# genome/ibwa

Hardware: AMD Instinct MI355X
Metric: reads/s `ibwa aln` GRCh37-sized 100bp, achieved HBM GB/s vs peak (higher is better)
Workload: dtype u32

## Files before the change

ibwa_amd/csrc/aln.hip:

```cpp
#include <hip/hip_runtime.h>
#include <stdint.h>
#include "engine.h"
#include "occ.h"

namespace ibwa {

namespace {


struct Fetch {
  uint4 ck, bk, sk, cl, bl, sl;
  uint32_t offk, offl;
  bool kneg;
};

__device__ __forceinline__ void fetch_pair(const IndexView &ix, uint32_t k, uint32_t l, Fetch &f) {
  f.kneg = (k == 0xFFFFFFFFu);
  uint32_t kk = f.kneg ? 0u : bwt_kk(ix, k);
  uint32_t ll = bwt_kk(ix, l);
  const uint4 *pk = ix.blk + (size_t)(kk >> 7) * 4;
  const uint4 *pl = ix.blk + (size_t)(ll >> 7) * 4;
  f.offk = kk & 127;
  f.offl = ll & 127;
  f.ck = pk[0];
// ... 84 lines not shown
}

__device__ __forceinline__ void occ4x2_from(const Fetch &f, uint32_t ck[4], uint32_t cl[4]) {
  if (f.kneg) {
    ck[0] = ck[1] = ck[2] = ck[3] = 0;
  } else {
    occ4_from(f.ck, f.bk, f.sk, f.offk, ck);
  }
  occ4_from(f.cl, f.bl, f.sl, f.offl, cl);
}

__device__ __forceinline__ uint32_t strand_base(uint32_t c, int a, bool comp) {
  return (a == 1 && comp && c < 4) ? 3u - c : c;
}

struct RecOut {
  uint32_t *words;
  uint32_t off, acc;
  __device__ __forceinline__ void put(uint32_t byte) {
    acc |= byte << (8 * (off & 3));
    if ((off & 3) == 3) {
      words[off >> 2] = acc;
      acc = 0;
    }
    ++off;
  }
  __device__ __forceinline__ void flush() {
    if (off & 3) words[off >> 2] = acc;
    acc = 0;
  }
};

__device__ __forceinline__ uint32_t rec_byte(uint2 a, uint2 b, uint32_t pa, uint32_t pb, bool first, uint32_t clamp,
                                             int nb) {
  const uint32_t ea = !first && a.x == pa, eb = !first && b.x == pb;
  return (a.y < clamp ? a.y : clamp) | ea << (nb - 1) | ((b.y < clamp ? b.y : clamp) | eb << (nb - 1)) << nb;
}

struct WChain {
  uint32_t k, l, bid;
  uint32_t mode, t, wi, w, w2;
};

struct WLoad {
  Fetch1 f;
  uint32_t q, w, w2, wi;
  bool tl;
};

__device__ __forceinline__ bool win_has(const WChain &h, uint32_t p) {
  return h.wi != 0xFFFFFFFFu && p >= 16u * h.wi && p - 16u * h.wi < 32u;
}

__device__ __forceinline__ void wchain_load(const IndexView &ix, const uint32_t *sa, const uint32_t *tx,
                                            const WChain &h, uint32_t c, WLoad &x, bool refresh) {
  fetch1(ix, h.k - 1, h.l, c & 3, c < 4 && h.mode != 2, x.f);
  x.q = 0;
  if (h.mode == 1) x.q = sa[h.k];
  const uint32_t p = h.t - 1u;
  x.tl = h.mode == 2 && h.t > 0 && (!win_has(h, p) || (refresh && !win_has(h, p >= 15u ? p - 15u : 0u)));
  x.wi = (p >= 15u ? p - 15u : 0u) >> 4;
  x.w = h.w;
  x.w2 = h.w2;
  if (x.tl) {
    x.w = tx[x.wi];
    x.w2 = tx[x.wi + 1];
  }
}

__device__ __forceinline__ void wchain_step(const IndexView &ix, bool jump, WChain &h, uint32_t c, const WLoad &x) {
  if (h.mode == 2) {
    if (x.tl) { h.w = x.w; h.w2 = x.w2; h.wi = x.wi; }
    const uint32_t p = h.t - 1u;
    const uint32_t tw = p - 16u * h.wi < 16u ? h.w : h.w2;
    if (h.t > 0 && c < 4 && ((tw >> (2 * (p & 15))) & 3u) == c) {
      --h.t;
    } else {
      h.k = 0; h.l = ix.seq_len; ++h.bid; h.mode = 0;
    }
    return;
  }
  bool reset = c > 3;
  if (c < 4) {
    uint32_t ok, ol;
    occ2_from1(x.f, c, ok, ol);
    h.k = l2of(ix, c) + ok + 1;
    h.l = l2of(ix, c) + ol;
    reset = h.k > h.l;
  }
  if (reset) { h.k = 0; h.l = ix.seq_len; ++h.bid; }
  if (h.mode == 1) {
    h.mode = reset ? 0u : 2u;
    h.t = x.q - 1u;
    h.wi = 0xFFFFFFFFu;
  } else if (jump && !reset && h.k == h.l) {
    h.mode = 1;
  }
}

__device__ __forceinline__ void width_pair(const IndexView ixa, const IndexView ixb, int L, const uint8_t *s, bool comp,
                                           uint2 *wa, uint2 *wb, uint32_t *lw = nullptr, RecOut *rec = nullptr,
                                           uint32_t clamp = 0, int nb = 4, uint32_t *rd = nullptr,
                                           const uint32_t *sa0 = nullptr, const uint32_t *sa1 = nullptr,
                                           const uint32_t *tx0 = nullptr, const uint32_t *tx1 = nullptr,
                                           const uint2 *lta = nullptr, const uint2 *ltb = nullptr, int tdep = 0) {
  WChain A{0u, ixa.seq_len, 0u, 0u, 0u, 0xFFFFFFFFu, 0u, 0u};
  WChain B{0u, ixb.seq_len, 0u, 0u, 0u, 0xFFFFFFFFu, 0u, 0u};
  uint32_t lwa = 0, lwb = 0;
  uint32_t pa = 0, pb = 0;
  constexpr int TMAX = 15;
  uint2 ta[TMAX], tb[TMAX];
  int da = 0, db = 0;
  if (tdep > 0) {
    const int D = L < tdep ? L : tdep;
    uint32_t xa = 0, xb = 0;
    int dn = D;
#pragma unroll
    for (int d = 0; d < TMAX; ++d) {
      ta[d] = tb[d] = make_uint2(1u, 0u);
      if (d < dn) {
// ... 14 lines not shown
      da += (d < dn && ta[d].x <= ta[d].y) ? 1 : 0;
      db += (d < dn && tb[d].x <= tb[d].y) ? 1 : 0;
    }
  }
  auto block = [&](int base, auto first) __attribute__((always_inline)) {
    constexpr bool FIRST = decltype(first)::value;
    uint2 ba[16], bb[16];
#pragma unroll
    for (int t = 0; t < 16; ++t) {
      const int i = base + t;
      if (i < L) {
        uint32_t ca = s[i];
        uint32_t cb = strand_base(ca, 1, comp);
        const bool tA = FIRST && t < TMAX && t < da, tB = FIRST && t < TMAX && t < db;
        WLoad xa, xb;
        if (!tA) wchain_load(ixa, sa0, tx0, A, ca, xa, t == 0);
        if (!tB) wchain_load(ixb, sa1, tx1, B, cb, xb, t == 0);
        if (FIRST && t < TMAX && tA) {
          A.k = ta[t < TMAX ? t : 0].x;
          A.l = ta[t < TMAX ? t : 0].y;
          if (t == da - 1 && sa0 != nullptr && A.k == A.l) A.mode = 1;
        } else {
          wchain_step(ixa, sa0 != nullptr, A, ca, xa);
        }
        if (FIRST && t < TMAX && tB) {
          B.k = tb[t < TMAX ? t : 0].x;
          B.l = tb[t < TMAX ? t : 0].y;
          if (t == db - 1 && sa1 != nullptr && B.k == B.l) B.mode = 1;
        } else {
          wchain_step(ixb, sa1 != nullptr, B, cb, xb);
        }
        ba[t] = make_uint2(A.l - A.k + 1, A.bid);
        lwa += 31 - __builtin_clz(A.l - A.k + 1);
        bb[t] = make_uint2(B.l - B.k + 1, B.bid);
        lwb += 31 - __builtin_clz(B.l - B.k + 1);
      }
    }
#pragma unroll
    for (int t = 0; t < 16; ++t)
      if (base + t < L) wa[base + t] = ba[t];
#pragma unroll
    for (int t = 0; t < 16; ++t)
      if (base + t < L) wb[base + t] = bb[t];
    if (rec) {
      uint32_t x = 0;
#pragma unroll
      for (int t = 0; t < 16; ++t)
        if (base + t < L) {
          rec->put(rec_byte(ba[t], bb[t], pa, pb, base + t == 0, clamp, nb));
          pa = ba[t].x;
          pb = bb[t].x;
          x |= ((uint32_t)s[base + t] & 3u) << (2 * t);
        }
      if (rd) rd[base >> 4] = x;
    }
  };
  if (L > 0) block(0, std::true_type{});
  for (int base = 16; base < L; base += 16) block(base, std::false_type{});
  wa[L] = make_uint2(0u, A.bid + 1);
  wb[L] = make_uint2(0u, B.bid + 1);
  if (rec) rec->put(rec_byte(wa[L], wb[L], pa, pb, L == 0, clamp, nb));
  if (lw) {
    lw[0] = lwa;
    lw[1] = lwb;
    lw[2] = A.bid;
    lw[3] = B.bid;
  }
}

__global__ void __launch_bounds__(256) k_width(AlnArgs A) {
  const int64_t lane = (int64_t)blockIdx.x * blockDim.x + threadIdx.x;
  if (lane >= A.n) return;
  const int64_t r = A.ids ? A.ids[lane] : lane;
  const int L = (int)A.len[r];
  const uint8_t *s = A.seq + A.off[r];
  const bool comp = A.o.mode & MODE_COMPREAD;
  const uint32_t *sa0 = A.jsa[0], *sa1 = A.jsa[1], *tx0 = A.jtxt[0], *tx1 = A.jtxt[1];
  const int tdep = A.ltab[0] ? (int)min(A.tab_k + 1u, 15u) : 0;
  uint2 *w0 = A.wbuf + (uint64_t)lane * A.wstride;
  uint2 *w1 = w0 + A.wlen1;
  uint2 *sw0 = w1 + A.wlen1;
  uint2 *sw1 = sw0 + (A.o.seed_len + 1);
  if (A.nN) {
    uint32_t nN = 0;
    for (int j = 0; j < L; ++j) nN += s[j] > 3;
    A.nN[lane] = (uint16_t)(nN > 0xFFFFu ? 0xFFFFu : nN);
  }
  if (A.feat) {
    uint32_t f[4] = {0, 0, 0, 0}, g[4] = {0, 0, 0, 0};
    width_pair(A.ix[0], A.ix[1], L, s, comp, w0, w1, f);
    if (L > A.o.seed_len) width_pair(A.ix[0], A.ix[1], A.o.seed_len, s + (L - A.o.seed_len), comp, sw0, sw1, g);
    A.feat[lane * 4 + 0] = (uint16_t)(f[0] + f[1]);
    A.feat[lane * 4 + 1] = (uint16_t)(g[0] + g[1]);
    A.feat[lane * 4 + 2] = (uint16_t)(f[2] < f[3] ? f[2] : f[3]);
    A.feat[lane * 4 + 3] = (uint16_t)(g[2] < g[3] ? g[2] : g[3]);
    return;
  }
  if (A.cw) {
    uint32_t *rec = A.cw + (uint64_t)lane * A.cw_words;
    uint32_t nN = 0;
    for (int j = 0; j < L; ++j) nN += s[j] > 3;
    const int md = A.o.fnr_pos ? (int)A.maxdiff_tab[L] : A.o.max_diff;
    rec[0] = (uint32_t)L | (nN < 255u ? nN : 255u) << 16 | (uint32_t)md << 24;
    RecOut ro{rec + 1 + A.cw_rw, 0u, 0u};
    width_pair(A.ix[0], A.ix[1], L, s, comp, w0, w1, nullptr, &ro, (uint32_t)md + 1u, 4, rec + 1, sa0, sa1, tx0, tx1,
               A.ltab[0], A.ltab[1], tdep);
    while (ro.off < A.wlen1) ro.put(0u);
    if (L > A.o.seed_len)
      width_pair(A.ix[0], A.ix[1], A.o.seed_len, s + (L - A.o.seed_len), comp, sw0, sw1, nullptr, &ro,
                 (uint32_t)A.o.max_seed_diff + 1u, 3, nullptr, sa0, sa1, tx0, tx1, A.ltab[0], A.ltab[1], tdep);
    ro.flush();
    return;
  }
  width_pair(A.ix[0], A.ix[1], L, s, comp, w0, w1, nullptr, nullptr, 0, 4, nullptr, sa0, sa1, tx0, tx1, A.ltab[0],
             A.ltab[1], tdep);
  if (L > A.o.seed_len)
    width_pair(A.ix[0], A.ix[1], A.o.seed_len, s + (L - A.o.seed_len), comp, sw0, sw1, nullptr, nullptr, 0, 4,
               nullptr, sa0, sa1, tx0, tx1, A.ltab[0], A.ltab[1], tdep);
}

__device__ __forceinline__ bool match_exact_alt(const IndexView &ix, int i, const uint8_t *s, int a, bool comp,
                                                uint32_t &k0, uint32_t &l0) {
  uint32_t k = k0, l = l0;
  for (int j = i - 1; j >= 0; --j) {
    uint32_t c = strand_base(s[j], a, comp);
    if (c > 3) return false;
    Fetch1 f;
    fetch1(ix, k - 1, l, c, true, f);
    uint32_t ok, ol;
    occ2_from1(f, c, ok, ol);
    k = l2of(ix, c) + ok + 1;
    l = l2of(ix, c) + ol;
    if (k > l) return false;
// ... 213 lines not shown
  int64_t t = (int64_t)blockIdx.x * blockDim.x + threadIdx.x;
  if (t >= n) return;
  uint32_t o[4];
  occ4(ix, k[t], o);
  cnt[4 * t + 0] = o[0];
  cnt[4 * t + 1] = o[1];
  cnt[4 * t + 2] = o[2];
  cnt[4 * t + 3] = o[3];
}

}

hipError_t launch_width(const AlnArgs &a, int block, hipStream_t st) {
  if (a.n <= 0) return hipSuccess;
  uint64_t grid = (a.n + block - 1) / block;
  hipLaunchKernelGGL(k_width, dim3((unsigned)grid), dim3(block), 0, st, a);
  return hipGetLastError();
}

hipError_t launch_search(const AlnArgs &a, int block, hipStream_t st) {
  if (a.n <= 0) return hipSuccess;
  uint64_t grid = (a.n + block - 1) / block;
  hipLaunchKernelGGL(k_search, dim3((unsigned)grid), dim3(block), 0, st, a);
  return hipGetLastError();
}

hipError_t launch_occ4(const IndexView &ix, int64_t n, const uint32_t *k, uint32_t *cnt, hipStream_t st) {
  if (n <= 0) return hipSuccess;
  hipLaunchKernelGGL(k_occ4, dim3((unsigned)((n + 255) / 256)), dim3(256), 0, st, ix, n, k, cnt);
  return hipGetLastError();
}
// ... 3 lines not shown
```

ibwa_amd/csrc/engine.h:

```cpp
#pragma once
#include <hip/hip_runtime.h>
#include <stdint.h>
#include "occ.h"

namespace ibwa {

constexpr uint32_t NIL = 0xFFFFFFFFu;
constexpr uint32_t ST_STACK_OVERFLOW = 1u;
constexpr uint32_t ST_ALN_OVERFLOW = 2u;
constexpr uint32_t ST_BAD_SCORE = 4u;
constexpr uint32_t ST_HEAVY = 8u;

enum CounterSlot {
  CTR_CLAIM = 0,
  CTR_STREAM = 1,
  CTR_WIDE_STREAM = 2,
  CTR_HANDED_ON = 3,
  CTR_RESUMED = 5,
  CTR_TAIL_JUMPS = 7,
};
enum CoopNextSlot {
  CNEXT_POOL = 0,
  CNEXT_PSTORE = 1,
};

struct AlnOpt {
  int s_mm, s_gapo, s_gape, mode;
  int indel_end_skip, max_del_occ, max_entries;
  int fnr_pos;
  int max_diff;
  int max_gapo;
  int max_gape, max_seed_diff, seed_len, max_top2;
  int n_stacks;
// ... 16 lines not shown
  uint4 *ent;
  uint32_t *prev;
  uint32_t cap;
  uint4 *aln;
  int32_t *n_aln;
  uint32_t aln_cap;
  uint32_t *status;
  uint16_t *nN;
  uint16_t *feat;
  uint32_t *cw;
  uint32_t cw_words, cw_rw;
  const uint32_t *jsa[2];
  const uint32_t *jtxt[2];
  const uint2 *ltab[2];
  uint32_t tab_k;
  AlnOpt o;
};

struct GapArgs {
  IndexView ix[2];
  const uint4 *o64[2];
  const uint8_t *seq;
  const uint64_t *off;
  const uint32_t *len;
  const int64_t *ids;
  int64_t n;
  int out_by_id;
  const int16_t *maxdiff_tab;
  uint2 *wbuf;
  uint64_t wstride;
// ... 267 lines not shown
```

ibwa_amd/csrc/engine_aln.hip:

```cpp
#include <hip/hip_runtime.h>
#include <stdio.h>
#include <string.h>
#include <sys/mman.h>

#include <algorithm>
#include <chrono>
#include <thread>
#include <vector>

#include "engine_ctx.h"

using namespace ibwa;

namespace {

void note_coop_pages(ibwa_ctx *c, uint32_t pool_pages) {
  uint32_t used = 0;
  if (hipMemcpy(&used, c->coop.c_next.as<uint32_t>() + CNEXT_POOL, 4, hipMemcpyDeviceToHost) != hipSuccess) return;
  c->stats.coop_pages_peak = std::max<int64_t>(c->stats.coop_pages_peak, std::min<uint32_t>(used, pool_pages));
  c->stats.coop_pages_cap = std::max<int64_t>(c->stats.coop_pages_cap, pool_pages);
}

GapArgs gap_args(const ibwa_ctx *c, const AlnArgs &A, const AlnOpt &o, int64_t b0, int64_t cnt) {
  GapArgs G = {};
// ... 120 lines not shown

  R.exact_path = c->exact_path && !o.fnr_pos && opt->max_diff == 0 && opt->max_entries >= 2;
  c->stats.path = R.exact_path ? 1 : 0;
  if (R.exact_path) return 0;

  R.v2 = c->gapped_v2 && batch_md + 1 <= 31 && o.max_gapo <= 7 && o.max_gape <= 15 &&
         gapped_lds_bytes(o.n_stacks, 64, true, 0, 0, 1, 4096) <= 65536 && max_len <= 65535;
  c->res.stream_out = R.v2;
  c->pass.hpop_valid = false;
  c->res.resumed_ids.clear();
  c->stats.n_resumed = 0;
  c->stats.resume_records = 0;
  c->stats.resume_records_peak = c->stats.resume_records_cap = 0;
  c->stats.coop_pages_peak = c->stats.coop_pages_cap = 0;
  c->stats.n_tail_jumps = 0;
  A.cap = c->stack_cap;
  return 0;
}

int exact_pass(Run &R) {
  ibwa_ctx *c = R.c;
  AlnArgs &A = R.A;
  const int64_t n = R.n;
  const int max_len = R.max_len;
  c->res.stream_out = false;
  A.aln_cap = c->aln_cap;
  A.n = n;
  if (int rc = c->pass.d_aln.ensure(std::max<int64_t>(n, 1) * (uint64_t)A.aln_cap * 16)) return rc;
  if (int rc = c->pass.d_naln.ensure(std::max<int64_t>(n, 1) * 4)) return rc;
  if (int rc = c->pass.d_status.ensure(std::max<int64_t>(n, 1) * 4)) return rc;
// ... 282 lines not shown
          (double)pf[20] / cnt, (double)pf[21] / cnt, pf[22] / li, pf[22]);
  return 0;
}

int first_pass_persistent(Run &R) {
  ibwa_ctx *c = R.c;
  AlnArgs &A = R.A;
  const AlnOpt &o = R.o;
  const int64_t n = R.n;
  if (int rc = ensure_kmer(c)) return rc;
  c->stats.path = 2;
  if (c->width_tab && c->index.ltab_K > 0 && c->index.ix[0].seq_len < LTAB_MARK) {
    A.ltab[0] = c->index.ltab[0].as<uint2>();
    A.ltab[1] = c->index.ltab[1].as<uint2>();
    A.tab_k = (uint32_t)c->index.ltab_K;
  }
  const FirstPassPlan P = plan_first_pass(R);
  const bool lw = P.lw, resume = P.resume;
  const int64_t chunk = P.chunk;
  if (int rc = c->pass.d_wbuf.ensure(chunk * A.wstride * 8)) return rc;
  if (int rc = c->pass.d_nN.ensure(chunk * 2 + 2)) return rc;
  if (lw) {
    if (int rc = c->pass.d_cw.ensure(chunk * (uint64_t)P.cw_words * 4)) return rc;
    if (int rc = c->pass.d_ptabg.ensure(P.lanes * GAP_MAX_PAGES * 2)) return rc;
  }
  if (resume) {
    if (int rc = c->pass.d_rdump.ensure(P.rd_cap * 16)) return rc;
    c->stats.resume_records_cap = (int64_t)P.rd_cap;
    if (int rc = c->pass.d_roff.ensure(((uint64_t)n + 4) * 8)) return rc;
    HIPCHK(zero_async(c->pass.d_roff.p, ((uint64_t)n + 4) * 8, c->stream));
    if (int rc = c->pass.d_hpop.ensure(((uint64_t)n + 1) * 4)) return rc;
    HIPCHK(zero_async(c->pass.d_hpop.p, ((uint64_t)n + 1) * 4, c->stream));
    R.resume_states = true;
    c->pass.hpop_valid = true;
  }
  if (int rc = c->pass.d_ent.ensure(P.lanes * P.P0r * 16)) return rc;
  if (int rc = c->pass.d_pool.ensure((uint64_t)P.blocks * P.ppb_run * (16ull << LG))) return rc;
  if (int rc = c->pass.d_aln.ensure(P.aln_total * 16)) return rc;
  if (int rc = c->pass.d_aoff.ensure(std::max<int64_t>(n, 1) * 8)) return rc;
  if (int rc = c->pass.d_naln.ensure(std::max<int64_t>(n, 1) * 4)) return rc;
  if (int rc = c->pass.d_status.ensure(std::max<int64_t>(n, 1) * 4)) return rc;
  if (int rc = c->d_counter.ensure(64)) return rc;
  HIPCHK(zero_async(counter(c, CTR_STREAM), 8, c->stream));
  HIPCHK(zero_async(counter(c, CTR_TAIL_JUMPS), 8, c->stream));
  for (int64_t b0 = 0; b0 < n; b0 += chunk) {
    const int64_t cnt = std::min(chunk, n - b0);
    AlnArgs B = A;
    B.n = cnt;
    B.off = A.off + b0;
    B.len = A.len + b0;
    B.wbuf = c->pass.d_wbuf.as<uint2>();
    B.nN = c->pass.d_nN.as<uint16_t>();
    GapArgs G = gap_args(c, A, o, b0, cnt);
    G.wbuf = B.wbuf;
    G.nN = B.nN;
    if (lw) {
      B.cw = c->pass.d_cw.as<uint32_t>();
      B.cw_words = P.cw_words;
      B.cw_rw = P.cw_rw;
// ... 35 lines not shown
      G.tail_iters = c->gap_tail_iters;
    }
    if (c->verbose || c->diag) {
      if (int rc = c->pass.d_iters.ensure(std::max<int64_t>(n, 1) * 4)) return rc;
      G.iters = c->pass.d_iters.as<uint32_t>() + b0;
    }
    if (c->diag) {
      if (int rc = c->pass.d_feat.ensure(std::max<int64_t>(n, 1) * 8)) return rc;
      B.feat = c->pass.d_feat.as<uint16_t>() + b0 * 4;
    }
    if (c->prof_phases) {
      if (int rc = c->d_prof.ensure(256)) return rc;
      HIPCHK(hipMemsetAsync(c->d_prof.p, 0, 256, c->stream));
      G.prof = c->d_prof.as<unsigned long long>();
    }
    HIPCHK(hipEventRecord(c->ev[0], c->stream));
    HIPCHK(launch_width(B, c->block, c->stream));
    HIPCHK(hipEventRecord(c->ev[1], c->stream));
    HIPCHK(launch_gapped(G, counter(c, CTR_CLAIM), P.blocks, P.block, false, c->stream));
    HIPCHK(hipEventRecord(c->ev[2], c->stream));
    HIPCHK(hipEventSynchronize(c->ev[2]));
    float a = 0, b = 0;
    HIPCHK(hipEventElapsedTime(&a, c->ev[0], c->ev[1]));
    HIPCHK(hipEventElapsedTime(&b, c->ev[1], c->ev[2]));
    R.ms_w += a;
    R.ms_s += b;
    c->stats.n_launch_width++;
    c->stats.n_launch_search++;
    if (c->verbose)
      if (int rc = print_gapped_iters(G.iters, cnt, b)) return rc;
    if (c->prof_phases)
      if (int rc = print_gapped_phases(c, P.blocks * P.block / 64, cnt)) return rc;
    if (R.resume_states)
// ... 442 lines not shown
  std::sort(patch.begin(), patch.end(), [](const auto &x, const auto &y) { return x.first < y.first; });
  c->res.patch_ids.resize(patch.size());
  c->res.patch_alns.resize(patch.size());
  for (size_t j = 0; j < patch.size(); ++j) {
    c->res.patch_ids[j] = patch[j].first;
    c->res.patch_alns[j].swap(patch[j].second);
  }
  c->res.retry_pass.swap(R.found_by);
  if (R.v2 && R.n) {
    HIPCHK(hipMemcpyAsync(&c->res.stream_len, counter(c, CTR_STREAM), 8, hipMemcpyDeviceToHost, c->stream));
    HIPCHK(hipStreamSynchronize(c->stream));
    c->res.stream_len = std::min<unsigned long long>(c->res.stream_len, c->res.stream_total);
    unsigned long long tj = 0;
    HIPCHK(hipMemcpy(&tj, counter(c, CTR_TAIL_JUMPS), 8, hipMemcpyDeviceToHost));
    c->stats.n_tail_jumps = (int64_t)tj;
  }
  c->stats.ms_retry = R.ms_r + R.res_ms;
  c->stats.n_retry = (int64_t)c->res.retry_ids.size() + R.res_ok;
  c->stats.ms_total = R.since();
  c->stats.ms_alloc = g_alloc_ms;
  return 0;
}

}

extern "C" {

int ibwa_batch_run(ibwa_ctx_t *c, const ibwa_gap_opt_t *opt, int batch_max_len) {
  Run R;
  R.c = c;
// ... 7 lines not shown
  if (int rc = wide_general_rounds(R)) return rc;
  return finish_run(R);
}

int ibwa_batch_retry_info(const ibwa_ctx_t *c, int64_t *ids, uint8_t *pass, int64_t cap, int64_t *n) {
  const int64_t m0 = (int64_t)c->res.retry_ids.size(), m = m0 + (int64_t)c->res.resumed_ids.size();
  for (int64_t j = 0; j < std::min(m, cap); ++j) {
    if (ids) ids[j] = j < m0 ? c->res.retry_ids[j] : c->res.resumed_ids[j - m0];
    if (pass) pass[j] = j >= m0 ? 4 : j < (int64_t)c->res.retry_pass.size() ? c->res.retry_pass[j] : 0;
  }
  if (n) *n = m;
  return 0;
}

int ibwa_batch_diag(const ibwa_ctx_t *c, int what, void *out, uint64_t cap_bytes) {
  if (what == 2) {
    const uint64_t need2 = (uint64_t)c->batch.n * 4;
    if (cap_bytes < need2) return fail(IBWA_EINVAL, "diag buffer too small");
    if (!c->pass.hpop_valid || c->pass.d_hpop.cap < need2) {
      memset(out, 0, need2);
      return 0;
    }
    if (c->batch.n == 0) return 0;
    HIPCHK(enter(c));
    HIPCHK(hipMemcpy(out, c->pass.d_hpop.p, need2, hipMemcpyDeviceToHost));
    return 0;
  }
  const uint64_t need = what == 0 ? (uint64_t)c->batch.n * 4 : (uint64_t)c->batch.n * 8;
  if (!c->diag || (what != 0 && what != 1)) return fail(IBWA_EINVAL, "set option diag=1 before the run; what = 0 or 1");
  if (cap_bytes < need) return fail(IBWA_EINVAL, "diag buffer too small");
// ... 151 lines not shown
```

ibwa_amd/csrc/engine_context.hip:

```cpp
#include <hip/hip_runtime.h>
#include <math.h>
#include <stdarg.h>
#include <stdio.h>
#include <string.h>

#include <algorithm>
#include <atomic>
#include <chrono>
#include <mutex>
#include <string>

#include "arena.h"
#include "engine_ctx.h"

using namespace ibwa;

namespace ibwa {

thread_local std::string g_err;
thread_local double g_alloc_ms = 0;
thread_local hipStream_t g_stream = nullptr;

int fail(int code, const char *fmt, ...) {
  char buf[512];
// ... 254 lines not shown
  else if (k == "gap_resume" && (value == 0 || value == 1)) c->gap_resume = (int)value;
  else if (k == "gap_resume_gb" && value >= 1 && value <= 256) c->gap_resume_gb = (int)value;
  else if (k == "gap_resume_records" && value >= 0) c->gap_resume_records = (int64_t)value;
  else if (k == "gap_resume_iters" && value >= 0) c->gap_resume_iters = (uint32_t)value;
  else if (k == "gap_resume_entries" && value >= 0) c->gap_resume_entries = (uint32_t)value;
  else if (k == "gap_tail_lanes" && value >= 0 && value <= 64) c->gap_tail_lanes = (uint32_t)value;
  else if (k == "gap_tail_iters" && value >= 0) c->gap_tail_iters = (uint32_t)value;
  else if (k == "gap_resume_ppb" && value >= 1 && value <= 65536) c->gap_resume_ppb = (int)value;
  else if (k == "gap_resume_cap1" && value >= 16 && value <= 65536) c->gap_resume_cap1 = (uint32_t)value;
  else if (k == "coop_roots" && (value == 0 || value == 1)) c->coop_roots = (int)value;
  else if (k == "gap_stream_per_read" && value >= 0 && value <= 4096) c->gap_stream_per_read = (uint32_t)value;
  else if (k == "gap_stream_min" && value >= 1) c->gap_stream_min = (uint64_t)value;
  else if (k == "exact_jump") c->exact_jump = value != 0;
  else if (k == "jump_derive") c->jump_derive = value != 0;
  else if (k == "width_jump" && value >= 0 && value <= 2) c->width_jump = (int)value;
  else if (k == "width_tab" && (value == 0 || value == 1)) c->width_tab = (int)value;
  else if (k == "gap_tail_tab" && (value == 0 || value == 1)) c->gap_tail_tab = (int)value;
  else if (k == "diag") c->diag = value != 0;
  else if (k == "sa_walk") c->sa_walk = value != 0;
  else if (k == "gap_coop") c->gap_coop = value != 0;
  else if (k == "coop_early" && (value == 0 || value == 1)) c->coop_early = (int)value;
  else if (k == "coop_waves_per_cu" && value > 0 && value <= 16) c->coop_waves_per_cu = (int)value;
  else if (k == "coop_pool_gb" && value >= 0 && value <= 256) c->coop_pool_gb = (int)value;
  else if (k == "coop_stg_room" && value >= 1 && value <= 4) c->coop_stg_room = (int)value;
  else if (k == "coop_pool_pages" && value >= 0 && value <= (1l << 24)) c->coop_pool_pages = (uint32_t)value;
  else if (k == "gap_resume_recs" && value >= 1 && value <= 65536) c->gap_resume_recs = (uint32_t)value;
  else if (k == "sw_stop" && value >= 0 && value <= 2) c->sw_stop_after = (int)value;
  else return fail(IBWA_EINVAL, "unknown option %s", k.c_str());
  return 0;
}

// ... 12 lines not shown
```

ibwa_amd/csrc/engine_ctx.h:

```cpp
#pragma once
#include <hip/hip_runtime.h>
#include <stdint.h>
#include <stdlib.h>

#include <string>
#include <vector>

#include "engine.h"
#include "ibwa_aln.h"

namespace ibwa {

extern thread_local std::string g_err;
int fail(int code, const char *fmt, ...) __attribute__((format(printf, 2, 3)));

#define HIPCHK(x)                                                                                    \
  do {                                                                                               \
    hipError_t e_ = (x);                                                                             \
    if (e_ != hipSuccess) return fail(IBWA_EHIP, "%s:%d %s: %s", __FILE__, __LINE__, #x, hipGetErrorString(e_)); \
  } while (0)

extern thread_local double g_alloc_ms;
extern thread_local hipStream_t g_stream;

// ... 116 lines not shown
  std::vector<uint32_t> h_status;
  std::vector<uint4> h_aln;
  std::vector<int64_t> retry_ids;
  std::vector<int64_t> patch_ids;
  std::vector<std::vector<uint4>> patch_alns;
  std::vector<uint8_t> retry_pass;
  std::vector<int64_t> resumed_ids;
  std::vector<uint64_t> h_aoff;
  std::vector<int32_t> h_cnt;
  uint32_t aln_cap_used = 0;
  bool stream_out = false;
  unsigned long long stream_len = 0;
  unsigned long long stream_total = 0;
  bool naln_on_host = true;
  bool fetched = false;
};

struct PassScratch {
  DBuf d_wbuf, d_heads, d_ent, d_prev, d_aln, d_naln, d_status, d_tab, d_ids;
  DBuf r_aln, r_naln, r_status;
  DBuf d_nN, d_pool, d_aoff, r_aoff, d_iters;
  DBuf d_cw, d_ptabg;
  DBuf d_rdump, d_roff;
  DBuf d_hpop;
  bool hpop_valid = false;
  DBuf d_feat;
};

struct CoopBufs {
  DBuf c_stg, c_dir, c_free, c_pool, c_hits, c_next, c_recb, c_proot, c_pstore;
// ... 40 lines not shown
  ibwa_run_stats_t stats = {};
  ibwa_ctx *share_src = nullptr;
  int n_borrowers = 0;
  bool destroy_pending = false;
  DBuf fq_codes, fq_offk, fq_lenk;
  ibwa::FqScratch *fqs = nullptr;
  int64_t fq_kept = 0;
  double fq_ms = 0;
  ~ibwa_ctx() {
    if (fqs) fqs->unref();
  }

  int coop_roots = 1;
  int jump_derive = 1;
  int exact_jump = 1;
  int width_tab = 1;
  int gap_tail_tab = 1;
  int width_jump = 1;
  int sa_walk = 0;
  uint32_t stack_cap = 4096, aln_cap = 8;
  int block = 256;
  int64_t lanes_per_chunk = 1 << 18;
  int exact_path = 1;
  int exact_blocks = 2048;
  int n_cus = 256;
  int gapped_v2 = 1;
  int gap_blocks_per_cu = 3;
  uint32_t gap_cap1 = 8192;
  int gap_pages_per_block = 384;
  uint32_t gap_hit_slots = 256;
  int64_t gap_reads_per_chunk = 1 << 24;
// ... 85 lines not shown
```

ibwa_amd/engine.py:

```python
import ctypes
import os
import struct

import numpy as np

from . import _native

c = ctypes


class GapOpt(c.Structure):
    _fields_ = [(n, c.c_int) for n in ("s_mm", "s_gapo", "s_gape", "mode", "indel_end_skip",
                                       "max_del_occ", "max_entries")] + \
               [("fnr", c.c_float)] + \
               [(n, c.c_int) for n in ("max_diff", "max_gapo", "max_gape", "max_seed_diff",
                                       "seed_len", "n_threads", "max_top2", "trim_qual")]


class RunStats(c.Structure):
    _fields_ = [("ms_width", c.c_double), ("ms_search", c.c_double), ("ms_retry", c.c_double),
                ("ms_total", c.c_double), ("n_retry", c.c_int64), ("n_launch_width", c.c_int64),
                ("n_launch_search", c.c_int64), ("path", c.c_int), ("kmer_k", c.c_int),
                ("n_stack_overflow", c.c_int64), ("n_aln_overflow", c.c_int64), ("n_heavy", c.c_int64), ("ms_sw", c.c_double),
                ("n_coop", c.c_int64), ("ms_coop", c.c_double), ("ms_sa2pos", c.c_double),
                ("sa2pos_full", c.c_int), ("ms_coop_width", c.c_double), ("ms_coop_roots", c.c_double),
                ("n_resumed", c.c_int64), ("resume_records", c.c_int64),
                ("resume_records_peak", c.c_int64), ("resume_records_cap", c.c_int64),
                ("coop_pages_peak", c.c_int64), ("coop_pages_cap", c.c_int64), ("ms_alloc", c.c_double),
                ("n_tail_jumps", c.c_int64)]


class RefSeq(c.Structure):
    _fields_ = [("name", c.c_void_p), ("seq", c.c_void_p), ("rseq", c.c_void_p), ("qual", c.c_void_p),
                ("len", c.c_uint32, 20), ("strand", c.c_uint32, 1), ("type", c.c_uint32, 2),
                ("dummy", c.c_uint32, 1), ("extra_flag", c.c_uint32, 8),
                ("n_mm", c.c_uint32, 8), ("n_gapo", c.c_uint32, 8), ("n_gape", c.c_uint32, 8),
                ("mapQ", c.c_uint32, 8), ("score", c.c_int), ("clip_len", c.c_int), ("n_aln", c.c_int),
                ("aln", c.c_void_p), ("n_multi", c.c_int), ("multi", c.c_void_p), ("sa", c.c_uint32),
                ("pos", c.c_uint64), ("remapped_pos", c.c_uint64), ("dbidx", c.c_uint32),
                ("remapped_dbidx", c.c_uint32), ("remapped_seqid", c.c_int32), ("remap_identical", c.c_int),
                ("c1", c.c_uint64, 28), ("c2", c.c_uint64, 28), ("seQ", c.c_uint64, 8), ("n_cigar", c.c_int),
                ("cigar", c.c_void_p), ("tid", c.c_int), ("bc", c.c_char * 16),
                ("full_len", c.c_uint32, 20), ("nm", c.c_uint32, 12), ("md", c.c_void_p)]

# ... 230 lines not shown
        _chk(lib().ibwa_batch_retry_info(self.h, ids.ctypes.data, ps.ctypes.data, n.value, c.byref(n)))
        return ids, ps

    def diag(self):
        it = np.zeros(self.n, np.uint32)
        ft = np.zeros((self.n, 4), np.uint16)
        _chk(lib().ibwa_batch_diag(self.h, 0, it.ctypes.data, it.nbytes))
        _chk(lib().ibwa_batch_diag(self.h, 1, ft.ctypes.data, ft.nbytes))
        return it, ft

    def handoff_pops(self):
        hp = np.zeros(self.n, np.uint32)
        _chk(lib().ibwa_batch_diag(self.h, 2, hp.ctypes.data, hp.nbytes))
        return hp

    @staticmethod
    def device_bytes():
        now, peak = c.c_int64(), c.c_int64()
        _chk(lib().ibwa_device_bytes(c.byref(now), c.byref(peak)))
        return now.value, peak.value

    def stats(self):
        st = RunStats()
        _chk(lib().ibwa_batch_stats(self.h, c.byref(st)))
        return st

    def aln(self, seqs, offs, lens, opt, batch_max_len=0):
        self.stage(seqs, offs, lens)
        self.run(opt, batch_max_len)
        return self.fetch()
# ... 280 lines not shown
```

include/ibwa_aln.h:

```cpp
#ifndef IBWA_ALN_H
#define IBWA_ALN_H
#include <stdint.h>

#ifdef __cplusplus
extern "C" {
#endif

enum {
	IBWA_OK = 0,
	IBWA_EHIP = -1,
	IBWA_EINVAL = -2,
	IBWA_ENOINDEX = -3,
	IBWA_EIO = -4,
	IBWA_EOVERFLOW = -5
};

typedef struct {
	int s_mm, s_gapo, s_gape;
	int mode;
	int indel_end_skip, max_del_occ, max_entries;
	float fnr;
	int max_diff, max_gapo, max_gape;
	int max_seed_diff, seed_len;
	int n_threads;
// ... 76 lines not shown
	double ms_sw;
	int64_t n_coop;
	double ms_coop;
	double ms_sa2pos;
	int sa2pos_full;
	double ms_coop_width;
	double ms_coop_roots;
	int64_t n_resumed;
	int64_t resume_records;
	int64_t resume_records_peak;
	int64_t resume_records_cap;
	int64_t coop_pages_peak;
	int64_t coop_pages_cap;
	double ms_alloc;
	int64_t n_tail_jumps;
} ibwa_run_stats_t;
int ibwa_batch_stats(const ibwa_ctx_t *ctx, ibwa_run_stats_t *st);

int ibwa_ctx_set_option(ibwa_ctx_t *ctx, const char *key, long value);

const char *ibwa_build_id(void);

int ibwa_aln_parse_args(int argc, char *const *argv, ibwa_gap_opt_t *opt, int *n_gpus, const char **fn_out);
int ibwa_aln_parse_args2(int argc, char *const *argv, ibwa_gap_opt_t *opt, int *n_gpus, const char **fn_out,
                         const char **fn_out2);

int ibwa_batch_retry_info(const ibwa_ctx_t *ctx, int64_t *ids, uint8_t *pass, int64_t cap, int64_t *n);

int ibwa_batch_diag(const ibwa_ctx_t *ctx, int what, void *out, uint64_t cap_bytes);

// ... 48 lines not shown
```

Before: 11.74 million.

## Stage width records in LDS for coalesced stores; add table restart after reset

Adds a mode in which each thread writes its compressed width record into a padded shared-memory tile. After a barrier the block copies the tile to global memory in a coalesced pattern, replacing strided per-lane global stores. It also adds a width-chain mode 3: after a reset, the next few bases are resolved with the precomputed k-mer lookup table instead of BWT occ fetches, and a step counter is gathered via a wave reduction and an atomic. Both are on by default (width_tab=2, width_rec_stage=1). The costs are extra LDS that may lower occupancy, a block barrier, and a new atomic.

```diff
diff --git a/ibwa_amd/csrc/aln.hip b/ibwa_amd/csrc/aln.hip
--- a/ibwa_amd/csrc/aln.hip
+++ b/ibwa_amd/csrc/aln.hip
@@ -122,19 +122,24 @@
   return (a == 1 && comp && c < 4) ? 3u - c : c;
 }
 
+template <bool STAGE>
 struct RecOut {
-  uint32_t *words;
+  using Ptr = typename std::conditional<STAGE, __attribute__((address_space(3))) uint32_t *, uint32_t *>::type;
+  Ptr words;
+  uint32_t stride;
+  uint32_t wb;
   uint32_t off, acc;
+  __device__ __forceinline__ void word(uint32_t w, uint32_t v) { words[STAGE ? w * stride : w] = v; }
   __device__ __forceinline__ void put(uint32_t byte) {
     acc |= byte << (8 * (off & 3));
     if ((off & 3) == 3) {
-      words[off >> 2] = acc;
+      word(wb + (off >> 2), acc);
       acc = 0;
     }
     ++off;
   }
   __device__ __forceinline__ void flush() {
-    if (off & 3) words[off >> 2] = acc;
+    if (off & 3) word(wb + (off >> 2), acc);
     acc = 0;
   }
 };
@@ -160,9 +165,11 @@
   return h.wi != 0xFFFFFFFFu && p >= 16u * h.wi && p - 16u * h.wi < 32u;
 }
 
+__device__ __forceinline__ uint32_t ltab_off32(uint32_t e) { return (0x55555555u >> (32u - 2u * e)) + 3u; }
+
 __device__ __forceinline__ void wchain_load(const IndexView &ix, const uint32_t *sa, const uint32_t *tx,
-                                            const WChain &h, uint32_t c, WLoad &x, bool refresh) {
-  fetch1(ix, h.k - 1, h.l, c & 3, c < 4 && h.mode != 2, x.f);
+                                            const uint2 *lt, const WChain &h, uint32_t c, WLoad &x, bool refresh) {
+  fetch1(ix, h.k - 1, h.l, c & 3, c < 4 && h.mode < 2, x.f);
   x.q = 0;
   if (h.mode == 1) x.q = sa[h.k];
   const uint32_t p = h.t - 1u;
@@ -174,9 +181,33 @@
     x.w = tx[x.wi];
     x.w2 = tx[x.wi + 1];
   }
-}
-
-__device__ __forceinline__ void wchain_step(const IndexView &ix, bool jump, WChain &h, uint32_t c, const WLoad &x) {
+  if (h.mode == 3) {
+    x.w = 1u;
+    x.w2 = 0u;
+    if (c < 4) {
+      const uint2 e = lt[ltab_off32(h.wi + 1u) + (h.t << 2 | c)];
+      x.w = e.x;
+      x.w2 = e.y;
+    }
+  }
+}
+
+__device__ __forceinline__ void wchain_step(const IndexView &ix, bool jump, uint32_t rdep, WChain &h, uint32_t c,
+                                            const WLoad &x, uint32_t &nt) {
+  if (h.mode == 3) {
+    ++nt;
+    if (x.w > x.w2) {
+      h.k = 0; h.l = ix.seq_len; ++h.bid; h.t = 0; h.wi = 0;
+      return;
+    }
+    h.k = x.w;
+    h.l = x.w2;
+    h.t = h.t << 2 | c;
+    ++h.wi;
+    if (jump && h.k == h.l) h.mode = 1;
+    else if (h.wi == rdep) h.mode = 0;
+    return;
+  }
   if (h.mode == 2) {
     if (x.tl) { h.w = x.w; h.w2 = x.w2; h.wi = x.wi; }
     const uint32_t p = h.t - 1u;
@@ -184,7 +215,8 @@
     if (h.t > 0 && c < 4 && ((tw >> (2 * (p & 15))) & 3u) == c) {
       --h.t;
     } else {
-      h.k = 0; h.l = ix.seq_len; ++h.bid; h.mode = 0;
+      h.k = 0; h.l = ix.seq_len; ++h.bid; h.mode = rdep ? 3u : 0u;
+      h.t = 0; h.wi = 0;
     }
     return;
   }
@@ -204,14 +236,18 @@
   } else if (jump && !reset && h.k == h.l) {
     h.mode = 1;
   }
-}
-
-__device__ __forceinline__ void width_pair(const IndexView ixa, const IndexView ixb, int L, const uint8_t *s, bool comp,
-                                           uint2 *wa, uint2 *wb, uint32_t *lw = nullptr, RecOut *rec = nullptr,
-                                           uint32_t clamp = 0, int nb = 4, uint32_t *rd = nullptr,
-                                           const uint32_t *sa0 = nullptr, const uint32_t *sa1 = nullptr,
-                                           const uint32_t *tx0 = nullptr, const uint32_t *tx1 = nullptr,
-                                           const uint2 *lta = nullptr, const uint2 *ltb = nullptr, int tdep = 0) {
+  if (reset && rdep) { h.mode = 3; h.t = 0; h.wi = 0; }
+}
+
+template <bool STAGE = false>
+__device__ __forceinline__ uint32_t width_pair(const IndexView ixa, const IndexView ixb, int L, const uint8_t *s, bool comp,
+                                               uint2 *wa, uint2 *wb, uint32_t *lw = nullptr,
+                                               RecOut<STAGE> *rec = nullptr, uint32_t clamp = 0, int nb = 4,
+                                               bool rd = false, const uint32_t *sa0 = nullptr,
+                                               const uint32_t *sa1 = nullptr, const uint32_t *tx0 = nullptr,
+                                               const uint32_t *tx1 = nullptr, const uint2 *lta = nullptr,
+                                               const uint2 *ltb = nullptr, int tdep = 0, uint32_t rdep = 0) {
+  uint32_t nt = 0;
   WChain A{0u, ixa.seq_len, 0u, 0u, 0u, 0xFFFFFFFFu, 0u, 0u};
   WChain B{0u, ixb.seq_len, 0u, 0u, 0u, 0xFFFFFFFFu, 0u, 0u};
   uint32_t lwa = 0, lwb = 0;
@@ -256,21 +292,21 @@
         uint32_t cb = strand_base(ca, 1, comp);
         const bool tA = FIRST && t < TMAX && t < da, tB = FIRST && t < TMAX && t < db;
         WLoad xa, xb;
-        if (!tA) wchain_load(ixa, sa0, tx0, A, ca, xa, t == 0);
-        if (!tB) wchain_load(ixb, sa1, tx1, B, cb, xb, t == 0);
+        if (!tA) wchain_load(ixa, sa0, tx0, lta, A, ca, xa, t == 0);
+        if (!tB) wchain_load(ixb, sa1, tx1, ltb, B, cb, xb, t == 0);
         if (FIRST && t < TMAX && tA) {
           A.k = ta[t < TMAX ? t : 0].x;
           A.l = ta[t < TMAX ? t : 0].y;
           if (t == da - 1 && sa0 != nullptr && A.k == A.l) A.mode = 1;
         } else {
-          wchain_step(ixa, sa0 != nullptr, A, ca, xa);
+          wchain_step(ixa, sa0 != nullptr, rdep, A, ca, xa, nt);
         }
         if (FIRST && t < TMAX && tB) {
           B.k = tb[t < TMAX ? t : 0].x;
           B.l = tb[t < TMAX ? t : 0].y;
           if (t == db - 1 && sa1 != nullptr && B.k == B.l) B.mode = 1;
         } else {
-          wchain_step(ixb, sa1 != nullptr, B, cb, xb);
+          wchain_step(ixb, sa1 != nullptr, rdep, B, cb, xb, nt);
         }
         ba[t] = make_uint2(A.l - A.k + 1, A.bid);
         lwa += 31 - __builtin_clz(A.l - A.k + 1);
@@ -294,7 +330,7 @@
           pb = bb[t].x;
           x |= ((uint32_t)s[base + t] & 3u) << (2 * t);
         }
-      if (rd) rd[base >> 4] = x;
+      if (rd) rec->word(1u + ((uint32_t)base >> 4), x);
     }
   };
   if (L > 0) block(0, std::true_type{});
@@ -308,17 +344,20 @@
     lw[2] = A.bid;
     lw[3] = B.bid;
   }
-}
-
-__global__ void __launch_bounds__(256) k_width(AlnArgs A) {
-  const int64_t lane = (int64_t)blockIdx.x * blockDim.x + threadIdx.x;
-  if (lane >= A.n) return;
+  return nt;
+}
+
+extern __shared__ uint32_t wrec[];
+
+template <bool STAGE>
+__device__ __forceinline__ uint32_t width_lane(const AlnArgs &A, int64_t lane) {
   const int64_t r = A.ids ? A.ids[lane] : lane;
   const int L = (int)A.len[r];
   const uint8_t *s = A.seq + A.off[r];
   const bool comp = A.o.mode & MODE_COMPREAD;
   const uint32_t *sa0 = A.jsa[0], *sa1 = A.jsa[1], *tx0 = A.jtxt[0], *tx1 = A.jtxt[1];
   const int tdep = A.ltab[0] ? (int)min(A.tab_k + 1u, 15u) : 0;
+  const uint32_t rdep = A.tab_reset ? (uint32_t)tdep : 0u;
   uint2 *w0 = A.wbuf + (uint64_t)lane * A.wstride;
   uint2 *w1 = w0 + A.wlen1;
   uint2 *sw0 = w1 + A.wlen1;
@@ -328,37 +367,74 @@
     for (int j = 0; j < L; ++j) nN += s[j] > 3;
     A.nN[lane] = (uint16_t)(nN > 0xFFFFu ? 0xFFFFu : nN);
   }
-  if (A.feat) {
+  if (!STAGE && A.feat) {
     uint32_t f[4] = {0, 0, 0, 0}, g[4] = {0, 0, 0, 0};
-    width_pair(A.ix[0], A.ix[1], L, s, comp, w0, w1, f);
-    if (L > A.o.seed_len) width_pair(A.ix[0], A.ix[1], A.o.seed_len, s + (L - A.o.seed_len), comp, sw0, sw1, g);
+    width_pair<false>(A.ix[0], A.ix[1], L, s, comp, w0, w1, f);
+    if (L > A.o.seed_len) width_pair<false>(A.ix[0], A.ix[1], A.o.seed_len, s + (L - A.o.seed_len), comp, sw0, sw1, g);
     A.feat[lane * 4 + 0] = (uint16_t)(f[0] + f[1]);
     A.feat[lane * 4 + 1] = (uint16_t)(g[0] + g[1]);
     A.feat[lane * 4 + 2] = (uint16_t)(f[2] < f[3] ? f[2] : f[3]);
     A.feat[lane * 4 + 3] = (uint16_t)(g[2] < g[3] ? g[2] : g[3]);
-    return;
-  }
-  if (A.cw) {
-    uint32_t *rec = A.cw + (uint64_t)lane * A.cw_words;
+    return 0;
+  }
+  if (STAGE || A.cw) {
+    RecOut<STAGE> ro;
+    if constexpr (STAGE) {
+      ro.words = (__attribute__((address_space(3))) uint32_t *)wrec + threadIdx.x;
+      ro.stride = blockDim.x + 1u;
+      for (uint32_t w = 0; w < A.cw_words; ++w) ro.word(w, 0u);
+    } else {
+      ro.words = A.cw + (uint64_t)lane * A.cw_words;
+      ro.stride = 1u;
+    }
+    ro.wb = 1u + A.cw_rw;
+    ro.off = ro.acc = 0u;
     uint32_t nN = 0;
     for (int j = 0; j < L; ++j) nN += s[j] > 3;
     const int md = A.o.fnr_pos ? (int)A.maxdiff_tab[L] : A.o.max_diff;
-    rec[0] = (uint32_t)L | (nN < 255u ? nN : 255u) << 16 | (uint32_t)md << 24;
-    RecOut ro{rec + 1 + A.cw_rw, 0u, 0u};
-    width_pair(A.ix[0], A.ix[1], L, s, comp, w0, w1, nullptr, &ro, (uint32_t)md + 1u, 4, rec + 1, sa0, sa1, tx0, tx1,
-               A.ltab[0], A.ltab[1], tdep);
+    ro.word(0u, (uint32_t)L | (nN < 255u ? nN : 255u) << 16 | (uint32_t)md << 24);
+    uint32_t nt = width_pair<STAGE>(A.ix[0], A.ix[1], L, s, comp, w0, w1, nullptr, &ro, (uint32_t)md + 1u, 4, true, sa0,
+                                    sa1, tx0, tx1, A.ltab[0], A.ltab[1], tdep, rdep);
     while (ro.off < A.wlen1) ro.put(0u);
     if (L > A.o.seed_len)
-      width_pair(A.ix[0], A.ix[1], A.o.seed_len, s + (L - A.o.seed_len), comp, sw0, sw1, nullptr, &ro,
-                 (uint32_t)A.o.max_seed_diff + 1u, 3, nullptr, sa0, sa1, tx0, tx1, A.ltab[0], A.ltab[1], tdep);
+      nt += width_pair<STAGE>(A.ix[0], A.ix[1], A.o.seed_len, s + (L - A.o.seed_len), comp, sw0, sw1, nullptr, &ro,
+                              (uint32_t)A.o.max_seed_diff + 1u, 3, false, sa0, sa1, tx0, tx1, A.ltab[0], A.ltab[1],
+                              tdep, rdep);
     ro.flush();
-    return;
-  }
-  width_pair(A.ix[0], A.ix[1], L, s, comp, w0, w1, nullptr, nullptr, 0, 4, nullptr, sa0, sa1, tx0, tx1, A.ltab[0],
-             A.ltab[1], tdep);
+    return nt;
+  }
+  uint32_t nt = width_pair<false>(A.ix[0], A.ix[1], L, s, comp, w0, w1, nullptr, nullptr, 0, 4, false, sa0, sa1, tx0, tx1,
+                           A.ltab[0], A.ltab[1], tdep, rdep);
   if (L > A.o.seed_len)
-    width_pair(A.ix[0], A.ix[1], A.o.seed_len, s + (L - A.o.seed_len), comp, sw0, sw1, nullptr, nullptr, 0, 4,
-               nullptr, sa0, sa1, tx0, tx1, A.ltab[0], A.ltab[1], tdep);
+    nt += width_pair<false>(A.ix[0], A.ix[1], A.o.seed_len, s + (L - A.o.seed_len), comp, sw0, sw1, nullptr, nullptr, 0, 4,
+                     false, sa0, sa1, tx0, tx1, A.ltab[0], A.ltab[1], tdep, rdep);
+  return nt;
+}
+
+template <bool STAGE>
+__global__ void __launch_bounds__(256) k_width(AlnArgs A) {
+  const int64_t lane0 = (int64_t)blockIdx.x * blockDim.x;
+  const int64_t lane = lane0 + threadIdx.x;
+  uint32_t nt = lane < A.n ? width_lane<STAGE>(A, lane) : 0u;
+  if constexpr (STAGE) {
+    __syncthreads();
+    const uint32_t cw = A.cw_words, bd = blockDim.x;
+    const int64_t left = A.n - lane0;
+    const uint32_t total = (uint32_t)(left < (int64_t)bd ? left : (int64_t)bd) * cw;
+    uint32_t *dst = A.cw + (uint64_t)lane0 * cw;
+    const uint32_t dq = bd / cw, dr = bd % cw;
+    uint32_t q = threadIdx.x / cw, w = threadIdx.x % cw;
+    for (uint32_t i = threadIdx.x; i < total; i += bd) {
+      dst[i] = wrec[w * (bd + 1u) + q];
+      q += dq;
+      w += dr;
+      if (w >= cw) { w -= cw; ++q; }
+    }
+  }
+  if (A.tab_steps) {
+    for (int o = 32; o > 0; o >>= 1) nt += __shfl_xor(nt, o);
+    if ((threadIdx.x & 63u) == 0 && nt) atomicAdd(A.tab_steps, (unsigned long long)nt);
+  }
 }
 
 __device__ __forceinline__ bool match_exact_alt(const IndexView &ix, int i, const uint8_t *s, int a, bool comp,
@@ -602,7 +678,12 @@
 hipError_t launch_width(const AlnArgs &a, int block, hipStream_t st) {
   if (a.n <= 0) return hipSuccess;
   uint64_t grid = (a.n + block - 1) / block;
-  hipLaunchKernelGGL(k_width, dim3((unsigned)grid), dim3(block), 0, st, a);
+  const size_t lds = (size_t)a.cw_words * ((size_t)block + 1) * 4;
+  const size_t per_cu = (12 * 64 + (size_t)block - 1) / (size_t)block;
+  if (a.cw_stage && a.cw && !a.feat && block % 64 == 0 && lds <= (64u << 10) && lds * per_cu <= (160u << 10))
+    hipLaunchKernelGGL(k_width<true>, dim3((unsigned)grid), dim3(block), lds, st, a);
+  else
+    hipLaunchKernelGGL(k_width<false>, dim3((unsigned)grid), dim3(block), 0, st, a);
   return hipGetLastError();
 }
 
diff --git a/ibwa_amd/csrc/engine.h b/ibwa_amd/csrc/engine.h
--- a/ibwa_amd/csrc/engine.h
+++ b/ibwa_amd/csrc/engine.h
@@ -17,6 +17,7 @@
   CTR_WIDE_STREAM = 2,
   CTR_HANDED_ON = 3,
   CTR_RESUMED = 5,
+  CTR_WIDTH_TAB = 6,
   CTR_TAIL_JUMPS = 7,
 };
 enum CoopNextSlot {
@@ -63,6 +64,9 @@
   const uint32_t *jtxt[2];
   const uint2 *ltab[2];
   uint32_t tab_k;
+  uint32_t tab_reset;
+  unsigned long long *tab_steps;
+  uint32_t cw_stage;
   AlnOpt o;
 };
 
diff --git a/ibwa_amd/csrc/engine_aln.hip b/ibwa_amd/csrc/engine_aln.hip
--- a/ibwa_amd/csrc/engine_aln.hip
+++ b/ibwa_amd/csrc/engine_aln.hip
@@ -158,6 +158,7 @@
   c->stats.resume_records_peak = c->stats.resume_records_cap = 0;
   c->stats.coop_pages_peak = c->stats.coop_pages_cap = 0;
   c->stats.n_tail_jumps = 0;
+  c->stats.n_width_tab_steps = 0;
   A.cap = c->stack_cap;
   return 0;
 }
@@ -470,7 +471,9 @@
     A.ltab[0] = c->index.ltab[0].as<uint2>();
     A.ltab[1] = c->index.ltab[1].as<uint2>();
     A.tab_k = (uint32_t)c->index.ltab_K;
-  }
+    A.tab_reset = c->width_tab == 2;
+  }
+  A.cw_stage = (uint32_t)c->width_rec_stage;
   const FirstPassPlan P = plan_first_pass(R);
   const bool lw = P.lw, resume = P.resume;
   const int64_t chunk = P.chunk;
@@ -499,6 +502,11 @@
   if (int rc = c->d_counter.ensure(64)) return rc;
   HIPCHK(zero_async(counter(c, CTR_STREAM), 8, c->stream));
   HIPCHK(zero_async(counter(c, CTR_TAIL_JUMPS), 8, c->stream));
+  HIPCHK(zero_async(counter(c, CTR_WIDTH_TAB), 8, c->stream));
+  A.tab_steps = counter(c, CTR_WIDTH_TAB);
+  c->res.diag_w.clear();
+  c->res.diag_cw.clear();
+  c->res.diag_shape[0] = c->res.diag_shape[1] = c->res.diag_shape[2] = 0;
   for (int64_t b0 = 0; b0 < n; b0 += chunk) {
     const int64_t cnt = std::min(chunk, n - b0);
     AlnArgs B = A;
@@ -564,9 +572,24 @@
       HIPCHK(hipMemsetAsync(c->d_prof.p, 0, 256, c->stream));
       G.prof = c->d_prof.as<unsigned long long>();
     }
+    const bool keep_w = c->diag_width && b0 == 0;
+    if (keep_w) {
+      HIPCHK(hipMemsetAsync(B.wbuf, 0, (uint64_t)cnt * A.wstride * 8, c->stream));
+      if (lw) HIPCHK(hipMemsetAsync(B.cw, 0, (uint64_t)cnt * P.cw_words * 4, c->stream));
+    }
     HIPCHK(hipEventRecord(c->ev[0], c->stream));
     HIPCHK(launch_width(B, c->block, c->stream));
     HIPCHK(hipEventRecord(c->ev[1], c->stream));
+    if (keep_w) {
+      c->res.diag_w.resize((uint64_t)cnt * A.wstride);
+      c->res.diag_cw.resize(lw ? (uint64_t)cnt * P.cw_words : 0);
+      c->res.diag_shape[0] = (uint64_t)cnt;
+      c->res.diag_shape[1] = A.wstride;
+      c->res.diag_shape[2] = lw ? P.cw_words : 0;
+      HIPCHK(hipStreamSynchronize(c->stream));
+      HIPCHK(hipMemcpy(c->res.diag_w.data(), B.wbuf, c->res.diag_w.size() * 8, hipMemcpyDeviceToHost));
+      if (lw) HIPCHK(hipMemcpy(c->res.diag_cw.data(), B.cw, c->res.diag_cw.size() * 4, hipMemcpyDeviceToHost));
+    }
     HIPCHK(launch_gapped(G, counter(c, CTR_CLAIM), P.blocks, P.block, false, c->stream));
     HIPCHK(hipEventRecord(c->ev[2], c->stream));
     HIPCHK(hipEventSynchronize(c->ev[2]));
@@ -1039,6 +1062,10 @@
     unsigned long long tj = 0;
     HIPCHK(hipMemcpy(&tj, counter(c, CTR_TAIL_JUMPS), 8, hipMemcpyDeviceToHost));
     c->stats.n_tail_jumps = (int64_t)tj;
+    if (R.A.tab_steps) {
+      HIPCHK(hipMemcpy(&tj, counter(c, CTR_WIDTH_TAB), 8, hipMemcpyDeviceToHost));
+      c->stats.n_width_tab_steps = (int64_t)tj;
+    }
   }
   c->stats.ms_retry = R.ms_r + R.res_ms;
   c->stats.n_retry = (int64_t)c->res.retry_ids.size() + R.res_ok;
@@ -1076,6 +1103,14 @@
 }
 
 int ibwa_batch_diag(const ibwa_ctx_t *c, int what, void *out, uint64_t cap_bytes) {
+  if (what >= 3 && what <= 5) {
+    const void *src = what == 3 ? (const void *)c->res.diag_w.data()
+                      : what == 4 ? (const void *)c->res.diag_cw.data() : (const void *)c->res.diag_shape;
+    const uint64_t need3 = what == 3 ? c->res.diag_w.size() * 8 : what == 4 ? c->res.diag_cw.size() * 4 : 24;
+    if (cap_bytes < need3) return fail(IBWA_EINVAL, "diag buffer too small");
+    if (need3) memcpy(out, src, need3);
+    return 0;
+  }
   if (what == 2) {
     const uint64_t need2 = (uint64_t)c->batch.n * 4;
     if (cap_bytes < need2) return fail(IBWA_EINVAL, "diag buffer too small");
diff --git a/ibwa_amd/csrc/engine_context.hip b/ibwa_amd/csrc/engine_context.hip
--- a/ibwa_amd/csrc/engine_context.hip
+++ b/ibwa_amd/csrc/engine_context.hip
@@ -292,7 +292,9 @@
   else if (k == "exact_jump") c->exact_jump = value != 0;
   else if (k == "jump_derive") c->jump_derive = value != 0;
   else if (k == "width_jump" && value >= 0 && value <= 2) c->width_jump = (int)value;
-  else if (k == "width_tab" && (value == 0 || value == 1)) c->width_tab = (int)value;
+  else if (k == "width_tab" && value >= 0 && value <= 2) c->width_tab = (int)value;
+  else if (k == "width_rec_stage" && (value == 0 || value == 1)) c->width_rec_stage = (int)value;
+  else if (k == "diag_width") c->diag_width = value != 0;
   else if (k == "gap_tail_tab" && (value == 0 || value == 1)) c->gap_tail_tab = (int)value;
   else if (k == "diag") c->diag = value != 0;
   else if (k == "sa_walk") c->sa_walk = value != 0;
diff --git a/ibwa_amd/csrc/engine_ctx.h b/ibwa_amd/csrc/engine_ctx.h
--- a/ibwa_amd/csrc/engine_ctx.h
+++ b/ibwa_amd/csrc/engine_ctx.h
@@ -154,6 +154,9 @@
   unsigned long long stream_total = 0;
   bool naln_on_host = true;
   bool fetched = false;
+  std::vector<uint2> diag_w;
+  std::vector<uint32_t> diag_cw;
+  uint64_t diag_shape[3] = {0, 0, 0};
 };
 
 struct PassScratch {
@@ -224,7 +227,9 @@
   int coop_roots = 1;
   int jump_derive = 1;
   int exact_jump = 1;
-  int width_tab = 1;
+  int width_tab = 2;
+  int width_rec_stage = 1;
+  int diag_width = 0;
   int gap_tail_tab = 1;
   int width_jump = 1;
   int sa_walk = 0;
diff --git a/ibwa_amd/engine.py b/ibwa_amd/engine.py
--- a/ibwa_amd/engine.py
+++ b/ibwa_amd/engine.py
@@ -27,7 +27,7 @@
                 ("n_resumed", c.c_int64), ("resume_records", c.c_int64),
                 ("resume_records_peak", c.c_int64), ("resume_records_cap", c.c_int64),
                 ("coop_pages_peak", c.c_int64), ("coop_pages_cap", c.c_int64), ("ms_alloc", c.c_double),
-                ("n_tail_jumps", c.c_int64)]
+                ("n_tail_jumps", c.c_int64), ("n_width_tab_steps", c.c_int64)]
 
 
 class RefSeq(c.Structure):
@@ -288,6 +288,23 @@
         _chk(lib().ibwa_batch_diag(self.h, 2, hp.ctypes.data, hp.nbytes))
         return hp
 
+    def _width_shape(self):
+        sh = np.zeros(3, np.uint64)
+        _chk(lib().ibwa_batch_diag(self.h, 5, sh.ctypes.data, sh.nbytes))
+        return int(sh[0]), int(sh[1]), int(sh[2])
+
+    def width_rows(self):
+        n, ws, _ = self._width_shape()
+        w = np.zeros((n, ws, 2), np.uint32)
+        _chk(lib().ibwa_batch_diag(self.h, 3, w.ctypes.data, w.nbytes))
+        return w
+
+    def width_records(self):
+        n, _, cw = self._width_shape()
+        r = np.zeros((n if cw else 0, cw), np.uint32)
+        _chk(lib().ibwa_batch_diag(self.h, 4, r.ctypes.data, r.nbytes))
+        return r
+
     @staticmethod
     def device_bytes():
         now, peak = c.c_int64(), c.c_int64()
diff --git a/include/ibwa_aln.h b/include/ibwa_aln.h
--- a/include/ibwa_aln.h
+++ b/include/ibwa_aln.h
@@ -114,6 +114,7 @@
 	int64_t coop_pages_cap;
 	double ms_alloc;
 	int64_t n_tail_jumps;
+	int64_t n_width_tab_steps;
 } ibwa_run_stats_t;
 int ibwa_batch_stats(const ibwa_ctx_t *ctx, ibwa_run_stats_t *st);
 
```

Result: faster. 11.96 million (median of 6 runs) (+1.9%).
